# Intelligent-Microsystems-Lab/SNNQuantPrune

Hardware: AMD Instinct MI355X
Metric: samples/sec/node (DVS128 T=20, 4-bit/90%-pruned) (higher is better)
Workload: dtype fp6*fp4->f32 (integer-exact); 1 GPU; C3 topology: 3x(qconv3x3+BN+LIF+pool2) + qdense(32768->110)+LIF + vote, DVS128 128x128x2, T=20, bits 4/4/4/4, 90% pruned; batch_per_gpu=1024, global_batch=1024, frames=20, parallelism=dp1 (batch-sharded, all-gather logits)

## Files before the change

### include/snnqp.h

```cpp
#ifndef SNNQP_H_
#define SNNQP_H_

#include <stdint.h>

#ifdef __cplusplus
extern "C" {
#endif

typedef void *snnqp_stream_t;

enum {
  SNNQP_OK = 0,
  SNNQP_EINVAL = -1,
  SNNQP_EUNSUPPORTED = -2,
  SNNQP_EHIP = -3
};

enum { SNNQP_F32 = 0, SNNQP_U8 = 1, SNNQP_BITS = 2, SNNQP_EV1 = 3, SNNQP_EV4 = 4 };
enum { SNNQP_W_F32 = 0, SNNQP_W_I8 = 1 };
enum {
  SNNQP_NEURON_NONE = 0,
  SNNQP_NEURON_MULTI_STEP_LIF = 1,
  SNNQP_NEURON_PARAMETRIC_LEAKY_IF = 2,
  SNNQP_NEURON_LIF = 3
// ... 73 lines not shown
  int32_t pad_lo[3], pad_hi[3];
  int32_t in_dil[3];
  int32_t k_dil[3];
  int32_t groups;
} snnqp_conv3d_geom_t;

#define SNNQP_VERSION 507
int snnqp_version(void);
const char *snnqp_last_error(void);
const char *snnqp_build_flags(void);

int snnqp_set_conv_k16(int enabled);
int snnqp_set_event_half_group(int enabled);
int snnqp_conv_event_half_group(int in_type, int32_t T, const snnqp_conv_geom_t *g, const snnqp_weight_t *w,
                                const snnqp_neuron_t *nrn, int has_state, int pool, int x_max);

int snnqp_conv_out_shape(const snnqp_conv_geom_t *g, int32_t *OH, int32_t *OW);

int snnqp_quantize(int kind, const float *w, const float *mask, int64_t n,
                   int bits, float p0, float p1, float *fq_out,
                   int8_t *codes_out, int32_t *flags, snnqp_stream_t stream);
int snnqp_quantize_ex(int kind, const float *w, const float *mask, int64_t n,
                      int bits, int sign, float p0, float p1, float *fq_out,
                      int8_t *codes_out, int32_t *flags, snnqp_stream_t stream);

int snnqp_pack_codes_mfma(const int8_t *w, int64_t K, int32_t N, int32_t Npad,
                          int8_t *wt, snnqp_stream_t stream);

int snnqp_pack_codes_fp6(const int8_t *w, int64_t K, int32_t N, int32_t Npad, void *wt6,
                         snnqp_stream_t stream);
// ... 234 lines not shown
```

### snnquantprune_amd/_lib.py

```python

from __future__ import annotations

import ctypes
import os
from ctypes import (POINTER, Structure, c_char_p, c_float, c_int, c_int8,
                    c_int32, c_uint32, c_int64, c_void_p)

_HERE = os.path.dirname(os.path.abspath(__file__))
LIB_PATH = os.path.join(_HERE, "csrc", "libsnnqp.so")

ABI_VERSION = 507

F32, U8, BITS, EV1, EV4 = 0, 1, 2, 3, 4
W_F32, W_I8 = 0, 1
NEURON_NONE, NEURON_MULTI_STEP_LIF, NEURON_PARAMETRIC_LEAKY_IF, NEURON_LIF = 0, 1, 2, 3
SURR_FAST_SIGMOID, SURR_ATAN, SURR_SLAYER, SURR_SMOOTH_STEP, SURR_PIECEWISE_LINEAR = 0, 1, 2, 3, 4
Q_DUQ, Q_UNIFORM_STATIC, Q_PARAMETRIC_D, Q_PARAMETRIC_D_XMAX = 0, 1, 2, 3
IMPL_AUTO, IMPL_GENERIC, IMPL_MFMA = 0, 1, 2
FLAG_CODE_OVERFLOW, FLAG_MASK_NOT_BINARY = 1, 2
FLAG_NOT_INTEGER, FLAG_GT_ONE, FLAG_GT_127, FLAG_GT_15 = 4, 8, 16, 32
OK, EINVAL, EUNSUPPORTED, EHIP = 0, -1, -2, -3
STATUS_QUEUE_CORRUPT, STATUS_TICKET, STATUS_BOUND = 1, 2, 4


# ... 25 lines not shown

class Conv3dGeomT(Structure):
  _fields_ = ([(n, c_int32) for n in ("D", "H", "W", "Cin", "Cout", "KD", "KH", "KW")]
              + [(n, c_int32 * 3) for n in ("stride", "pad_lo", "pad_hi", "in_dil", "k_dil")]
              + [("groups", c_int32)])


_PROTOTYPES = {
    "snnqp_version": (c_int, []),
    "snnqp_last_error": (c_char_p, []),
    "snnqp_build_flags": (c_char_p, []),
    "snnqp_set_conv_k16": (c_int, [c_int]),
    "snnqp_set_event_half_group": (c_int, [c_int]),
    "snnqp_conv_event_half_group": (c_int, [c_int, c_int32, POINTER(ConvGeomT), POINTER(WeightT),
                                            POINTER(NeuronT), c_int, c_int, c_int]),
    "snnqp_conv_out_shape": (c_int, [POINTER(ConvGeomT), POINTER(c_int32),
                                     POINTER(c_int32)]),
    "snnqp_quantize": (c_int, [c_int, c_void_p, c_void_p, c_int64, c_int, c_float,
                               c_float, c_void_p, c_void_p, c_void_p, c_void_p]),
    "snnqp_quantize_ex": (c_int, [c_int, c_void_p, c_void_p, c_int64, c_int, c_int, c_float,
                                  c_float, c_void_p, c_void_p, c_void_p, c_void_p]),
    "snnqp_pack_codes_mfma": (c_int, [c_void_p, c_int64, c_int32, c_int32, c_void_p,
                                      c_void_p]),
    "snnqp_pack_codes_fp6": (c_int, [c_void_p, c_int64, c_int32, c_int32, c_void_p, c_void_p]),
    "snnqp_inspect_f32": (c_int, [c_void_p, c_int64, c_void_p, c_void_p]),
    "snnqp_inspect_u8": (c_int, [c_void_p, c_int64, c_void_p, c_void_p]),
    "snnqp_f32_to_u8": (c_int, [c_void_p, c_void_p, c_int64, c_void_p]),
    "snnqp_narrow_f32": (c_int, [c_void_p, c_void_p, c_int64, c_void_p, c_void_p]),
    "snnqp_pack_frames": (c_int, [c_void_p, c_int64, c_int32, c_int32, c_int, c_void_p, c_void_p,
                                  c_void_p]),
# ... 179 lines not shown
```

### snnquantprune_amd/csrc/api.hip

```cpp
#include <atomic>

#include "common.h"

namespace snnqp {

static std::atomic<int> g_conv_k16{1};
bool conv_k16_enabled() { return g_conv_k16.load(std::memory_order_relaxed) != 0; }
static std::atomic<int> g_event_half_group{1};
bool event_half_group_enabled() { return g_event_half_group.load(std::memory_order_relaxed) != 0; }

static thread_local std::string g_last_error;

void set_error(const char *fmt, ...) {
  char buf[512];
  va_list ap;
  va_start(ap, fmt);
  vsnprintf(buf, sizeof(buf), fmt, ap);
  va_end(ap);
  g_last_error = buf;
}

}

extern "C" {
// ... 5 lines not shown
#ifndef SNNQP_BUILD_FLAGS
#define SNNQP_BUILD_FLAGS ""
#endif
const char *snnqp_build_flags(void) { return SNNQP_BUILD_FLAGS; }

int snnqp_set_conv_k16(int enabled) {
  if (enabled < 0) return snnqp::conv_k16_enabled() ? 1 : 0;
  return snnqp::g_conv_k16.exchange(enabled ? 1 : 0, std::memory_order_relaxed);
}

int snnqp_set_event_half_group(int enabled) {
  if (enabled < 0) return snnqp::event_half_group_enabled() ? 1 : 0;
  return snnqp::g_event_half_group.exchange(enabled ? 1 : 0, std::memory_order_relaxed);
}

int snnqp_conv_out_shape(const snnqp_conv_geom_t *g, int32_t *OH, int32_t *OW) {
  SNNQP_REQUIRE(g && OH && OW, SNNQP_EINVAL, "conv_out_shape: null argument");
  SNNQP_REQUIRE(g->stride_h > 0 && g->stride_w > 0 && g->in_dil_h > 0 &&
                    g->in_dil_w > 0 && g->k_dil_h > 0 && g->k_dil_w > 0 &&
                    g->KH > 0 && g->KW > 0,
                SNNQP_EINVAL, "conv_out_shape: non-positive stride/dilation/kernel");
  const int64_t hd = g->H > 0 ? (int64_t)(g->H - 1) * g->in_dil_h + 1 : 0;
  const int64_t wd = g->W > 0 ? (int64_t)(g->W - 1) * g->in_dil_w + 1 : 0;
  const int64_t kh = (int64_t)(g->KH - 1) * g->k_dil_h + 1;
  const int64_t kw = (int64_t)(g->KW - 1) * g->k_dil_w + 1;
  const int64_t th = hd + g->pad_h_lo + g->pad_h_hi;
  const int64_t tw = wd + g->pad_w_lo + g->pad_w_hi;
  *OH = th < kh ? 0 : (int32_t)((th - kh) / g->stride_h + 1);
  *OW = tw < kw ? 0 : (int32_t)((tw - kw) / g->stride_w + 1);
  return SNNQP_OK;
// ... 4 lines not shown
```

### snnquantprune_amd/csrc/blocks.hip

```cpp
#include "common.h"
#include "kernels.h"

#include <atomic>
#include <cstdlib>
#include <cstring>
#include <mutex>

using namespace snnqp;

namespace {
std::atomic<int64_t> g_fallback_conv{0}, g_fallback_dense{0};
std::mutex g_fallback_mu;
char g_fallback_reason[256] = "";

void note_fallback(bool dense, const char *why) {
  (dense ? g_fallback_dense : g_fallback_conv).fetch_add(1, std::memory_order_relaxed);
  static const bool log = std::getenv("SNNQP_LOG_FALLBACKS") != nullptr;
  std::lock_guard<std::mutex> lock(g_fallback_mu);
  const bool fresh = std::strncmp(g_fallback_reason + (dense ? 7 : 6), why ? why : "", 200) != 0;
  std::snprintf(g_fallback_reason, sizeof(g_fallback_reason), "%s%s", dense ? "dense: " : "conv: ",
                why ? why : "");
  if (log && fresh)
    std::fprintf(stderr, "libsnnqp: %s block on the direct-form kernel: %s\n",
                 dense ? "dense" : "conv", why ? why : "");
// ... 65 lines not shown
  }
  return SNNQP_OK;
}

int snnqp_conv_dequant_form(const snnqp_weight_t *w, const snnqp_neuron_t *nrn) {
  SNNQP_REQUIRE(w && nrn, SNNQP_EINVAL, "conv_dequant_form: null descriptor");
  SNNQP_REQUIRE(w->wtype == SNNQP_W_I8, SNNQP_EINVAL, "conv_dequant_form: int8 codes only");
  return conv3x3_bits_dequant_form(w, nrn);
}

int snnqp_conv_event_half_group(int in_type, int32_t T, const snnqp_conv_geom_t *g, const snnqp_weight_t *w,
                                const snnqp_neuron_t *nrn, int has_state, int pool, int x_max) {
  SNNQP_REQUIRE(g && w && nrn, SNNQP_EINVAL, "conv_event_half_group: null descriptor");
  SNNQP_CHECK_NEURON_KIND(nrn, "conv_event_half_group");
  return conv3x3_event_half_group(in_type, T, g, w, nrn, has_state != 0, pool, x_max);
}

int snnqp_conv_lif_forward(const void *x, int in_type, int64_t x_stride_t,
                           int64_t x_stride_b, int32_t T, int32_t B,
                           const snnqp_conv_geom_t *g, const snnqp_weight_t *w,
                           const int8_t *wt, const snnqp_bn_t *bn,
                           const snnqp_neuron_t *nrn,
                           const float *u0, float *u_out, void *s_out,
                           int s_type, int pool, int impl, int x_max, int32_t *x_seen,
                           int32_t *x_flags, snnqp_stream_t stream) {
  const BlockCall c{x, in_type, x_stride_t, x_stride_b, T, B, w, wt, bn, nrn, u0, u_out, s_out, s_type,
                    x_flags, nullptr, (hipStream_t)stream, g, pool, x_max, x_seen};
  if (int rc = conv_preamble("conv_lif_forward", c, false, true)) return rc;
  SNNQP_REQUIRE(impl >= SNNQP_IMPL_AUTO && impl <= SNNQP_IMPL_MFMA, SNNQP_EINVAL,
                "conv_lif_forward: unknown impl %d", impl);
// ... 122 lines not shown
```

### snnquantprune_amd/csrc/conv3x3_u8c2.hip

```cpp
#include <type_traits>

#include "conv_tile.h"

namespace snnqp {

constexpr int HROW2 = 24;
constexpr int HCOPY2 = HALO * HROW2;
constexpr int HCONST2 = 2 * HCOPY2;
constexpr int HIMG2 = 496;
constexpr int TCHUNK = 32;
constexpr int U8C2_WPS = 4;
constexpr int STG_N = TCHUNK / 2;

typedef int v2i_a4 __attribute__((ext_vector_type(2), aligned(4)));
typedef __attribute__((address_space(3))) const v2i_a4 lds_cv2i_t;

__host__ __device__ inline int u8c2_table_bytes(int lutm, int bound, int rows) {
  const int b = lutm == LUT_CHANNEL ? rows * 128 : lutm == LUT_SHARED ? (2 * bound + 2) * 4 : 0;
  return (b + 15) & ~15;
}

#ifndef SNNQP_U8C2_EV1_WPS
#define SNNQP_U8C2_EV1_WPS 5
#endif
#ifndef SNNQP_U8C2_ONE_WPS
#define SNNQP_U8C2_ONE_WPS 4
#endif
#ifndef SNNQP_U8C2_EV1_ONE_WPS
#define SNNQP_U8C2_EV1_ONE_WPS 6
#endif
template <int NF, bool POOL, int LUTM, int IN, bool ONE>
constexpr int u8c2_waves() {
  if (IN == SNNQP_EV1 && ONE && LUTM == LUT_CHANNEL && NF == NF_MUL0 && POOL) return SNNQP_U8C2_EV1_ONE_WPS;
  if (IN == SNNQP_EV1) return SNNQP_U8C2_EV1_WPS;
  return ONE ? SNNQP_U8C2_ONE_WPS : U8C2_WPS;
}
template <int NF, bool POOL, int LUTM, int IN = SNNQP_U8, bool ONE = false, bool HALF = false>
__global__ void __launch_bounds__(256, (u8c2_waves<NF, POOL, LUTM, IN, ONE>()))
conv3x3_u8c2_kernel(ConvMfmaArgs a) {
  constexpr int FL = OutStage<POOL>::FL;
  constexpr bool EV1 = IN == SNNQP_EV1;
  static_assert(!HALF || (EV1 && ONE && LUTM == LUT_CHANNEL && NF == NF_MUL0),
                "the half group: bit-packed frames, one chunk, per-channel tables, NF_MUL0");
  constexpr bool EV4 = IN == SNNQP_EV4;
  constexpr bool F32IN = IN == SNNQP_F32;
  static_assert(TCHUNK % FL == 0, "flush period must divide the staging chunk");
  if constexpr (!EV1) {
    if (a.pred && *(const volatile int32_t *)a.pred == 0) return;
  }
  extern __shared__ __attribute__((aligned(16))) uint8_t lds[];
  const int tc = a.tchunk;
  const int lut_off = tc * HIMG2;
  uint32_t *obuf = (uint32_t *)(lds + lut_off + u8c2_table_bytes(LUTM, a.lut_bound, a.lut_rows));
  const int tid = threadIdx.x, lane = tid & 63;
  const int wave = __builtin_amdgcn_readfirstlane(tid >> 6);
  const int n = lane & 31, h = lane >> 5;
  const int cout_base = blockIdx.y * 128 + wave * 32;
  const bool wave_on = cout_base < a.Cout;
  const int cout = wave_on ? cout_base + n : n;
  const int cpar = cout < a.Cout ? cout : a.Cout - 1;
  const uint32_t cmask = chan_mask(cout_base, a.cout_fire);
  const bool half_wave = HALF && cout_base + 32 == a.Cout;
  const int ctab = half_wave && n >= 16 ? cout - 16 : cout;
  uint32_t *wgw = obuf + OutStage<POOL>::BYTES / 4;
  if (tid == 0) { wgw[0] = 0x7F800000u; wgw[1] = 0u; }
  typedef int v2i_a8 __attribute__((ext_vector_type(2)));
  v2i_a8 *xtab = (v2i_a8 *)(wgw + 4);
  if (EV1) {
    const uint32_t one = LUTM == LUT_CHANNEL ? 16u : LUTM == LUT_SHARED ? 4u : 0x81u;
    const uint32_t zero = LUTM == LUT_NONE ? 0x80u : 0u;
    uint32_t e[2] = {0, 0};
#pragma unroll
    for (int j = 0; j < 8; ++j) e[j >> 2] |= (((uint32_t)tid >> j) & 1u ? one : zero) << (8 * (j & 3));
    xtab[tid] = v2i_a8{(int)e[0], (int)e[1]};
  }
  if (LUTM != LUT_NONE) lds_barrier();
  if (LUTM == LUT_SHARED) {
    build_lut((float *)(lds + lut_off), a.lut_bound, a.dq, tid);
    if (NF == NF_MUL0) {
      lds_barrier();
      atomicMin(wgw, lut_bn_min_bits((const float *)(lds + lut_off), a.lut_bound, a.bn,
                                     blockIdx.y * 128, a.Cout, tid, 256));
    }
  }
  int ch_row0 = 0, ch_col = 0;
  if (LUTM == LUT_CHANNEL) {
    int pos = 0, neg = 0;
#pragma unroll
    for (int j = 0; j < 16; ++j) {
      const int k = 16 * h + j, dy = k >> 3, b = k & 7;
      if (k < 24 && b < 6 && wave_on && cout < a.Cout) {
        const int code = a.w[(int64_t)(6 * dy + b) * a.Cout + ctab];
        pos += code > 0 ? code : 0;
        neg += code < 0 ? -code : 0;
      }
    }
    pos += __shfl_xor(pos, 32);
    neg += __shfl_xor(neg, 32);
    uint32_t *scr = obuf;
    int slot = 4 * n + wave;
    if (a.ch_slots) slot = a.ch_slots[blockIdx.y * 128 + wave * 32 + n] & 127;
    if (h == 0) {
      scr[slot] = (uint32_t)((pos + neg) * a.x_limit + 1);
      scr[128 + wave * 32 + n] = (uint32_t)(neg * a.x_limit);
      scr[256 + wave * 32 + n] = (uint32_t)slot;
    }
    lds_barrier();
    ch_col = slot >> 2;
    const int start = lut_column_start(scr, slot);
    int total = 0;
#pragma unroll
    for (int k = 0; k < 4; ++k) total += (int)scr[(slot & ~3) + k];
    ch_row0 = start + neg * a.x_limit;
    if (total > a.lut_rows && a.status) *(volatile uint32_t *)a.status = SNNQP_STATUS_BOUND;
    const uint32_t mb = build_lut_channel<HALF>((float *)(lds + lut_off), scr, a.lut_rows, a.dq, a.bn,
                                                blockIdx.y * 128, a.Cout, tid);
    atomicMin(wgw, mb);
    lds_barrier();
  }
  if (tid < tc) {
    *(uint32_t *)(lds + tid * HIMG2 + HCONST2) = 0x7F7F7F7Fu;
    *(uint32_t *)(lds + tid * HIMG2 + HCONST2 + 4) = 0x00000001u;
  }

  float acc_off = 0.0f;
  int tab0 = 0;
  v4i bf, bfg;
  {
    int bias = 0;
    if (LUTM == LUT_SHARED) bias = (int)lds_addr(lds) + lut_off + 4 * a.lut_bound;
    if (LUTM == LUT_CHANNEL)
      bias = (int)lds_addr(lds) + lut_off + 4 * (ch_row0 * 32 + ch_col);
    if (HALF) tab0 = bias;
    int q = bias / 127;
    const int r = bias - 127 * q;
    int wsum = 0;
    int v[4], vg[4];
#pragma unroll
    for (int d = 0; d < 4; ++d) {
      uint32_t pk = 0, pkg = 0;
#pragma unroll
      for (int j = 0; j < 4; ++j) {
        const int k = 16 * h + 4 * d + j;
// ... 24 lines not shown
      vg[d] = (int)pkg;
    }
    bf = v4i{v[0], v[1], v[2], v[3]};
    bfg = v4i{vg[0], vg[1], vg[2], vg[3]};
    acc_off = 128.0f * (float)(wsum + __shfl_xor(wsum, 32));
  }

  LaneConsts lc = {0.f, 1.f, 0.f, 0.f, a.nrn.vr};
  if (a.bn.mean) { lc.bmean = a.bn.mean[cpar]; lc.bmul = a.bn.mul[cpar]; lc.bbias = a.bn.bias[cpar]; }
  if (a.nrn.kind == SNNQP_NEURON_LIF) lc.dec = a.nrn.decay[cpar];

  const int ty = ((n >> 2) & 1) | ((n >> 4) << 1);
  const int tx = (n & 3) | (((n >> 3) & 1) << 2);
  const int cpy = tx & 1;
  const int px0 = (int)lds_addr(lds) + cpy * HCOPY2 + 2 * tx + 2 * cpy;
  const int tyh = half_wave ? 2 * ty : ty;
  int offA[2], offB[2];
#pragma unroll
  for (int tl = 0; tl < 2; ++tl) {
    offA[tl] = px0 + (tyh + 4 * tl + (h ? 2 : 0)) * HROW2;
    offB[tl] = h ? (int)lds_addr(lds) + HCONST2 : px0 + (ty + 4 * tl + 1) * HROW2;
  }
  if (HALF && half_wave) offB[1] = tab0;
  const uint8_t *xb = (const uint8_t *)a.x;
  const int ob0 = (half_wave ? lane : out_pix<POOL>(0, lane)) * 4 + wave;
  const int ob1 = out_pix<POOL>(1, lane) * 4 + wave;
  const bool store_lane = POOL ? lane < (half_wave ? 16 : 8) : (half_wave || lane < 32);
  uint32_t seen = 0;
  uint32_t hist[6] = {0, 0, 0, 0, 0, 0};
  const int s_pix = tid & 127;
  const bool s_task = s_pix < HALO * HALO;
  const int s_half = __builtin_amdgcn_readfirstlane(tid >> 7);
  const int s_dst = (s_pix / HALO) * HROW2 + (s_pix % HALO) * 2;

  PatchWalk pw(a);
  int r = __builtin_amdgcn_readfirstlane((int)pw.first);
  uint32_t processed = 0;
  while (r < (int)pw.count) {
    ++processed;
    int claimed = 0;
    if (pw.queue && tid == 0) claimed = (int)pw.claim();
    int b, y0, x0;
// ... 140 lines not shown
            }
            const uint16_t val = (uint16_t)(w2 ^ 0x8080u);
            uint8_t *p = lds + tt * HIMG2 + s_dst;
            *(uint16_t *)p = val;
            *(uint16_t *)(p + HCOPY2 + 2) = val;
          }
        }
        lds_barrier();
      }
      }
      auto run_chunk = [&](auto mode_tag, auto fma_tag) {
      constexpr int MODE = decltype(mode_tag)::value;
      constexpr bool FMA = decltype(fma_tag)::value;
      constexpr bool OFFS = MODE == LUT_NONE;
      const v4i bw = OFFS ? bfg : bf;
      if constexpr (HALF) {
        if (half_wave) {
          int ctab0 = offB[1];
          asm volatile("" : "+v"(ctab0));
          const v16i c0 = splat16(ctab0);
          for (int tf = 0; tf < nt; tf += FL) {
            const int nf = min(FL, nt - tf);
#pragma unroll 1
            for (int tt = tf; tt < tf + nf; ++tt) {
              const uint32_t img = (uint32_t)(tt * HIMG2);
              const v2i_a4 lo = *(lds_cv2i_t *)(uintptr_t)(img + (uint32_t)offA[0]);
              const v2i_a4 hi = *(lds_cv2i_t *)(uintptr_t)(img + (uint32_t)offA[0] + (uint32_t)HROW2);
              const v16i acc = __builtin_amdgcn_mfma_i32_32x32x32_i8(v4i{lo.x, lo.y, hi.x, hi.y}, bw, c0,
                                                                     0, 0, 0);
              const uint32_t word = tile_epilogue_halves<NF, POOL, MODE, FMA, OFFS, true>(
                  acc, u[0], a.dq, lc, a.nrn, lane, acc_off);
              if (store_lane) {
// ... 60 lines not shown
    r = r_next;
  }
  if (a.x_seen && tid == 0) {
    if (seen != 0) atomicMax(a.x_seen, seen);
#pragma unroll
    for (int k = 0; k < 6; ++k)
      if (hist[k] != 0) atomicAdd((uint32_t *)a.x_seen + 1 + k, hist[k]);
  }
  if (pw.queue && tid == 0) pw.finish(processed, a.npatch, a.status);
}


namespace {
struct U8c2Plan {
  int32_t x_limit, lut_bound, lut_rows, tchunk;
  bool lut, lutc, one, half;
  size_t ldsb;
};
U8c2Plan u8c2_plan(int in_type, int32_t T, int32_t Cout, const snnqp_weight_t *w, int nf, bool has_state,
                   bool pl, int x_max) {
  U8c2Plan p;
  const bool ev1 = in_type == SNNQP_EV1;
  const int64_t xm = ev1 ? 1 : (x_max > 0 ? x_max : 1);
  p.x_limit = (int32_t)(xm > 255 ? 255 : xm);
  const int64_t bound = (int64_t)w->abs_sum_max * xm;
  p.lut = w->abs_sum_max > 0 && xm > 0 && xm <= LUT_XMAX && bound <= LUT_CAP;
  p.lut_bound = p.lut ? (int32_t)bound : 0;
  p.tchunk = T >= TCHUNK ? TCHUNK : T;
  const size_t lds_fixed = (size_t)p.tchunk * HIMG2 + 16 + (ev1 ? 2048 : 0) +
                           (pl ? OutStage<true>::BYTES : OutStage<false>::BYTES);
  const int64_t stack = w->ch_stack_max > 0 ? (int64_t)w->ch_stack_max : 8 * (int64_t)w->abs_sum_max;
// ... 3 lines not shown
  const int lm = p.lutc ? LUT_CHANNEL : p.lut ? LUT_SHARED : LUT_NONE;
  const size_t lds_rest = lds_fixed - (size_t)p.tchunk * HIMG2 + u8c2_table_bytes(lm, p.lut_bound, p.lut_rows);
  for (int wgs = 4; wgs >= 2; --wgs) {
    const size_t per_wg = (size_t)(160 * 1024) / wgs - 512;
    int tc = p.tchunk;
    while (tc > 16 && (size_t)tc * HIMG2 + lds_rest > per_wg) tc -= 1;
    if ((size_t)tc * HIMG2 + lds_rest <= per_wg) {
      p.tchunk = tc;
      break;
    }
  }
  p.ldsb = (size_t)p.tchunk * HIMG2 + lds_rest;
  p.one = !has_state && T <= p.tchunk;
  p.half = event_half_group_enabled() && ev1 && p.one && p.lutc && nf == NF_MUL0 && w->cout_fire > 0 &&
           w->cout_fire % 16 == 0 && w->cout_fire + 16 == Cout && Cout % 32 == 0;
  return p;
}
}

int conv3x3_event_half_group(int in_type, int32_t T, const snnqp_conv_geom_t *g, const snnqp_weight_t *w,
                             const snnqp_neuron_t *nrn, bool has_state, int pool, int x_max) {
  SNNQP_REQUIRE(g && w && nrn, SNNQP_EINVAL, "conv_event_half_group: null descriptor");
  SNNQP_REQUIRE(pool == 1 || pool == 2, SNNQP_EINVAL, "conv_event_half_group: pool must be 1 or 2");
  SNNQP_REQUIRE(T >= 0, SNNQP_EINVAL, "conv_event_half_group: negative T");
  if (in_type != SNNQP_EV1 || T == 0) return 0;
  BlockCall c;
  c.in_type = in_type; c.g = g; c.w = w; c.nrn = nrn;
  if (conv3x3_mfma_unsupported(c)) return 0;
  SNNQP_REQUIRE(w->L >= 1.0f, SNNQP_EINVAL, "dequant L must be >= 1");
  if (int rc = conv3x3_check_cout_fire("conv_event_half_group", w, g->Cout)) return rc;
  return u8c2_plan(in_type, T, g->Cout, w, neuron_form(make_neuron(nrn)), has_state, pool == 2, x_max).half ? 1 : 0;
}

template <int NF, int LUTM, int IN>
static void launch_u8c2_pool(const ConvMfmaArgs &a, bool pool, bool one, unsigned gy, hipStream_t st, size_t lds) {
  if (pool && one) launch_persistent(conv3x3_u8c2_kernel<NF, true, LUTM, IN, true>, a, gy, st, lds);
  else if (pool) launch_persistent(conv3x3_u8c2_kernel<NF, true, LUTM, IN>, a, gy, st, lds);
  else if (one) launch_persistent(conv3x3_u8c2_kernel<NF, false, LUTM, IN, true>, a, gy, st, lds);
  else launch_persistent(conv3x3_u8c2_kernel<NF, false, LUTM, IN>, a, gy, st, lds);
}

template <int NF, int LUTM>
static void launch_u8c2_in(const ConvMfmaArgs &a, int in_type, bool pool, bool one, unsigned gy, hipStream_t st,
                           size_t lds) {
  if (in_type == SNNQP_EV1) launch_u8c2_pool<NF, LUTM, SNNQP_EV1>(a, pool, one, gy, st, lds);
  else if (in_type == SNNQP_EV4) launch_u8c2_pool<NF, LUTM, SNNQP_EV4>(a, pool, one, gy, st, lds);
// ... 20 lines not shown
  const unsigned gy = (unsigned)((a.Cout + 127) / 128);
  const U8c2Plan plan = u8c2_plan(in_type, a.T, a.Cout, w, nf, a.u0 || a.u_out, pl, x_max);
  a.x_limit = plan.x_limit;
  a.lut_bound = plan.lut_bound;
  a.tchunk = plan.tchunk;
  a.lut_rows = plan.lut_rows;
  a.ch_slots = plan.lutc && w->ch_stack_max > 0 ? w->ch_slots : nullptr;
  a.cout_fire = w->cout_fire > 0 ? w->cout_fire : a.Cout;
  if (in_type == SNNQP_F32) {
    SNNQP_REQUIRE(x_flags != nullptr && (((uintptr_t)a.x) & 7) == 0 && a.xs_t % 2 == 0 && a.xs_b % 2 == 0,
                  SNNQP_EINVAL, "conv3x3 mfma: float32 frames need x_flags and 8-byte aligned pixels");
    if (int rc = zero_words_async((uint32_t *)x_flags, 1, st)) return rc;
    a.x_flags = x_flags;
  }
  if (plan.lut) check_code_bound_once(stream_device(st), a.w, (int64_t)9 * a.Cin, a.Cout, w->abs_sum_max, st);
  if (plan.half && pl)
    launch_persistent(conv3x3_u8c2_kernel<NF_MUL0, true, LUT_CHANNEL, SNNQP_EV1, true, true>, a, gy, st, plan.ldsb);
  else if (plan.half)
    launch_persistent(conv3x3_u8c2_kernel<NF_MUL0, false, LUT_CHANNEL, SNNQP_EV1, true, true>, a, gy, st, plan.ldsb);
  else if (plan.lutc) launch_u8c2_nf<LUT_CHANNEL>(a, nf, in_type, pl, plan.one, gy, st, plan.ldsb);
  else if (plan.lut) launch_u8c2_nf<LUT_SHARED>(a, nf, in_type, pl, plan.one, gy, st, plan.ldsb);
  else launch_u8c2_nf<LUT_NONE>(a, nf, in_type, pl, plan.one, gy, st, plan.ldsb);
  return SNNQP_OK;
}

}
```

### snnquantprune_amd/csrc/conv_tile.h

```cpp
#pragma once
#include "kernels.h"

namespace snnqp {

struct v2f {
  float x, y;
};
__device__ __forceinline__ v2f operator+(v2f a, v2f b) { return v2f{a.x + b.x, a.y + b.y}; }
__device__ __forceinline__ v2f operator-(v2f a, v2f b) { return v2f{a.x - b.x, a.y - b.y}; }
__device__ __forceinline__ v2f operator*(v2f a, v2f b) { return v2f{a.x * b.x, a.y * b.y}; }
__device__ __forceinline__ v2f operator+(v2f a, float b) { return v2f{a.x + b, a.y + b}; }
__device__ __forceinline__ v2f operator-(v2f a, float b) { return v2f{a.x - b, a.y - b}; }
__device__ __forceinline__ v2f operator*(v2f a, float b) { return v2f{a.x * b, a.y * b}; }
__device__ __forceinline__ v2f operator-(v2f a) { return v2f{-a.x, -a.y}; }
__device__ __forceinline__ v2f fma2(v2f a, v2f b, v2f c) {
  return v2f{__builtin_fmaf(a.x, b.x, c.x), __builtin_fmaf(a.y, b.y, c.y)};
}


enum { LUT_NONE = 0, LUT_SHARED = 1, LUT_CHANNEL = 2 };
constexpr int LUT_CAP = 4095;
constexpr int LUT2_ROWS = 256;
constexpr int LUT_XMAX = 31;

// ... 302 lines not shown
        const uint32_t pw = (uint32_t)o | (uint32_t)(o >> 32);
        myw = writelane_u32(pw, i >> 1, myw);
      } else {
        const int r0 = (i & 3) + 8 * (i >> 2);
        myw = writelane_u32((uint32_t)m0, r0, myw);
        myw = writelane_u32((uint32_t)(m0 >> 32), r0 + 4, myw);
        myw = writelane_u32((uint32_t)m1, r0 + 1, myw);
        myw = writelane_u32((uint32_t)(m1 >> 32), r0 + 5, myw);
      }
    }
    __builtin_amdgcn_sched_barrier(0);
  }
  return myw;
}

template <bool POOL>
struct OutStage {
  static constexpr int NPIX = POOL ? 16 : 64;
  static constexpr int FL = POOL ? 32 : 8;
  static constexpr int BYTES = FL * NPIX * 16;
};

template <bool POOL>
__device__ __forceinline__ int out_pix(int tl, int lane) {
  if (POOL) return (tl * 2 + ((lane >> 2) & 1)) * 4 + (lane & 3);
  const int ty = ((lane >> 2) & 1) | (((lane >> 4) & 1) << 1);
  const int tx = (lane & 3) | (((lane >> 3) & 1) << 2);
  return (tl * 4 + ty) * 8 + tx;
}

// ... 85 lines not shown
  const unsigned gx = persistent_grid((const void *)kernel, threads, dyn_lds, dev, a.npatch, a.B, &a.xcd_split);
  hipLaunchKernelGGL(kernel, dim3(gx, gy), dim3(threads), dyn_lds, st, a);
  if (a.sched) sched_release(dev, slot, st);
}

int conv3x3_check_cout_fire(const char *who, const snnqp_weight_t *w, int32_t Cout);
inline int wt_cin_pad(const snnqp_weight_t *w, int32_t Cin) { return w->wt_cin ? w->wt_cin : (Cin + 31) / 32 * 32; }

enum { DQ_ARITH = 1, DQ_ONE = 2, DQ_TABLE = 3 };
constexpr int DQT_MAXA = 2047;
void launch_conv3x3_bits(ConvMfmaArgs a, const snnqp_weight_t *w, const snnqp_neuron_t *nrn, hipStream_t st);
int launch_conv3x3_u8c2(ConvMfmaArgs a, int in_type, const snnqp_weight_t *w, int x_max, int32_t *x_flags,
                        hipStream_t st);
bool conv_k16_enabled();
bool event_half_group_enabled();

}
```

### snnquantprune_amd/csrc/kernels.h

```cpp
#pragma once
#include "common.h"
#include "tile_util.h"

namespace snnqp {

struct BlockCall {
  const void *x = nullptr;
  int in_type = SNNQP_BITS;
  int64_t xs_t = 0, xs_b = 0;
  int32_t T = 0, B = 0;
  const snnqp_weight_t *w = nullptr;
  const int8_t *wt = nullptr;
  const snnqp_bn_t *bn = nullptr;
  const snnqp_neuron_t *nrn = nullptr;
  const float *u0 = nullptr;
  float *u_out = nullptr;
  void *s_out = nullptr;
  int s_type = SNNQP_BITS;
  int32_t *x_flags = nullptr;
  const int32_t *pred = nullptr;
  hipStream_t st = nullptr;
  const snnqp_conv_geom_t *g = nullptr;
  int pool = 1, x_max = 0;
  int32_t *x_seen = nullptr;
// ... 17 lines not shown
};
int run_generic(const BlockCall &c, int32_t *acc_out, const GenericDepth *dz);

const char *conv3x3_geometry_unsupported(const snnqp_conv_geom_t *g);
const char *conv3x3_mfma_unsupported(const BlockCall &c);
const char *conv3x3_currents_unsupported(int in_type, int64_t NB, const snnqp_conv_geom_t *g,
                                         const snnqp_weight_t *w, const int8_t *wt);
int run_conv3x3_currents(const void *x, int64_t NB, const snnqp_conv_geom_t *g,
                         const snnqp_weight_t *w, const int8_t *wt, float *y, int32_t *acc,
                         hipStream_t st);
int run_current_min(const snnqp_weight_t *w, const snnqp_bn_t *bn, int32_t bound, int32_t Cout,
                    uint32_t *out_bits, hipStream_t st);
int conv3x3_bits_dequant_form(const snnqp_weight_t *w, const snnqp_neuron_t *nrn);
int conv3x3_event_half_group(int in_type, int32_t T, const snnqp_conv_geom_t *g, const snnqp_weight_t *w,
                             const snnqp_neuron_t *nrn, bool has_state, int pool, int x_max);
int run_conv3x3_mfma(const BlockCall &c);

constexpr int MAX_DEVICES = 64;
struct DeviceGuard {
  int prev = -1;
  bool ok = true;
  explicit DeviceGuard(int dev) {
    int cur = -1;
    if (hipGetDevice(&cur) != hipSuccess) { (void)hipGetLastError(); ok = false; return; }
    if (cur == dev) return;
    if (hipSetDevice(dev) != hipSuccess) { (void)hipGetLastError(); ok = false; return; }
    prev = cur;
  }
  ~DeviceGuard() {
    if (prev >= 0 && hipSetDevice(prev) != hipSuccess) (void)hipGetLastError();
// ... 42 lines not shown
```

### snnquantprune_amd/linen.py

```python

from __future__ import annotations

import dataclasses
import functools
import hashlib
import math
import threading
from collections.abc import MutableMapping
from typing import Any, Callable, Dict, Iterable, Optional, Sequence

import torch

_tls = threading.local()


def _stack():
  if not hasattr(_tls, "stack"):
    _tls.stack = []
  return _tls.stack


class ConfigDict(MutableMapping):

  def __init__(self, *args, **kwargs):
# ... 92 lines not shown


def conv_k16() -> bool:
  from . import _lib
  return bool(_lib.lib().snnqp_set_conv_k16(-1))


def set_event_half_group(enabled: bool):
  from . import _lib
  _lib.lib().snnqp_set_event_half_group(1 if enabled else 0)


def event_half_group() -> bool:
  from . import _lib
  return bool(_lib.lib().snnqp_set_event_half_group(-1))


_TRAIN_CONV_MFMA = True


def set_train_conv_mfma(enabled: bool) -> bool:
  global _TRAIN_CONV_MFMA
  old = _TRAIN_CONV_MFMA
  _TRAIN_CONV_MFMA = bool(enabled)
  return old


def train_conv_mfma() -> bool:
  return _TRAIN_CONV_MFMA

# ... 458 lines not shown
```

### snnquantprune_amd/ops.py

```python

from __future__ import annotations

import ctypes
import math
from dataclasses import dataclass
from typing import Optional, Sequence, Tuple

import torch

from . import _lib as L




class PackedSpikes:

  def __init__(self, bits: torch.Tensor, channels: int):
    assert bits.dtype == torch.int32 and bits.is_contiguous()
    assert bits.shape[-1] == (channels + 31) // 32
    self.bits = bits
    self.channels = int(channels)
    self.flat_perm = None
    self.chan_map = None

# ... 935 lines not shown
  dev = xt.device
  u0, u_out, s, spikes = _scan_outputs(dev, (T, B, OH // pool, OW // pool), geom.Cout, u0, want_u, packed_out,
                               state=(B, OH, OW))
  g, w, n = geom.struct(), weight.struct(), neuron.struct()
  b = bn.struct() if bn is not None else None
  cin_l, cout_l = (geom.Cin, geom.Cout) if logical is None else logical[:2]
  tag = "conv%dx%d[%dx%dx%d->%d]" % (geom.KH, geom.KW, geom.H, geom.W, cin_l, cout_l)
  if _PROFILE is not None and in_type == L.BITS and weight.is_int and "dequant" not in PROFILE_NOTES.get(tag, {}):
    PROFILE_NOTES.setdefault(tag, {})["dequant"] = conv_dequant_form(weight, neuron)
  if _PROFILE is not None and logical is not None:
    PROFILE_NOTES.setdefault(tag, {})["channels"] = {
        "cin": geom.Cin, "cout": geom.Cout, "live_out": int(logical[2])}
    if weight.cout_fire and packed_out:
      ev1 = L.EV1 if (in_type == L.EV1 or (binary_first and in_type in (L.U8, L.F32))) else in_type
      PROFILE_NOTES[tag]["channels"]["half_group"] = conv_event_half_group(
          ev1, T, geom, weight, neuron, state=u0 is not None or want_u, pool=pool, x_max=1 if ev1 == L.EV1 else x_max)
  speculate = (binary_first and packed_out and not isinstance(x, (PackedFrames, PackedSpikes))
               and in_type in (L.U8, L.F32) and geom.Cin == 2 and weight.is_int and impl != L.IMPL_GENERIC
               and xt.ndim == 5)
  with _timed(tag):
    if speculate:
      pf, not_binary = pack_frames_checked(xt)
      ps_t, ps_b = _tb_strides(pf.data, T, B, time_major, pf.data.shape[-1])
      try:
        L.check(L.lib().snnqp_conv_lif_forward(
            _ptr(pf.data), L.EV1, ps_t, ps_b, T, B, ctypes.byref(g), ctypes.byref(w),
            _ptr(weight.wt), _ref(b), ctypes.byref(n),
            _ptr(u0), _ptr(u_out), _ptr(s), L.BITS, pool, impl, 1, None, None, _stream()))
      except L.SnnqpError as e:
        if e.code != L.EUNSUPPORTED:
# ... 144 lines not shown
  L.check(L.lib().snnqp_workqueue_stats(ctypes.byref(a), ctypes.byref(b), ctypes.byref(c), 1 if reset else 0))
  return {"captured_static_walks": a.value, "busy_static_walks": b.value, "dequant_table_fallbacks": c.value}


def workqueue_capture_mark(device) -> int:
  m = ctypes.c_int64()
  L.check(L.lib().snnqp_workqueue_capture_mark(int(torch.device(device).index or 0), ctypes.byref(m)))
  return int(m.value)


def workqueue_capture_release(device, begin: int, end: int):
  L.check(L.lib().snnqp_workqueue_capture_release(int(torch.device(device).index or 0), int(begin), int(end)))


DQ_FORMS = {1: "arith", 2: "one", 3: "table"}


def conv_event_half_group(in_type: int, T: int, geom: ConvGeom, w: Weight, nrn: Neuron, state: bool = False,
                          pool: int = 1, x_max: int = 0) -> bool:
  gs, ws, ns = geom.struct(), w.struct(), nrn.struct()
  rc = L.lib().snnqp_conv_event_half_group(int(in_type), int(T), ctypes.byref(gs), ctypes.byref(ws),
                                           ctypes.byref(ns), 1 if state else 0, int(pool), int(x_max))
  if rc < 0:
    L.check(rc)
  return rc == 1


def conv_dequant_form(w: Weight, nrn: Neuron) -> str:
  ws, ns = w.struct(), nrn.struct()
  rc = L.lib().snnqp_conv_dequant_form(ctypes.byref(ws), ctypes.byref(ns))
# ... 494 lines not shown
```

Measured before the change: 98080 samples/s.

## Spread first-layer event conv work across all waves instead of idling tail waves

Adds a 'wave spread' variant of the bit-packed-frame first conv kernel. When Cout is 64, or 96 with the half group, each wave pair now covers one 32-channel group and splits the two row tiles between its two waves. The extra 16-channel half group is also split into quarter tiles across all four waves, so no wave idles or loops twice. The intent is to balance MFMA and epilogue work across waves in the CTA, removing the imbalance where the half wave did double work. The cost is extra per-wave weight-fragment construction, a new quarter epilogue, and a different occupancy bound.

```diff
diff --git a/include/snnqp.h b/include/snnqp.h
--- a/include/snnqp.h
+++ b/include/snnqp.h
@@ -111,6 +111,9 @@
 int snnqp_set_event_half_group(int enabled);
 int snnqp_conv_event_half_group(int in_type, int32_t T, const snnqp_conv_geom_t *g, const snnqp_weight_t *w,
                                 const snnqp_neuron_t *nrn, int has_state, int pool, int x_max);
+int snnqp_set_event_wave_spread(int enabled);
+int snnqp_conv_event_wave_spread(int in_type, int32_t T, const snnqp_conv_geom_t *g, const snnqp_weight_t *w,
+                                 const snnqp_neuron_t *nrn, int has_state, int pool, int x_max);
 
 int snnqp_conv_out_shape(const snnqp_conv_geom_t *g, int32_t *OH, int32_t *OW);
 
diff --git a/snnquantprune_amd/_lib.py b/snnquantprune_amd/_lib.py
--- a/snnquantprune_amd/_lib.py
+++ b/snnquantprune_amd/_lib.py
@@ -63,6 +63,9 @@
     "snnqp_set_event_half_group": (c_int, [c_int]),
     "snnqp_conv_event_half_group": (c_int, [c_int, c_int32, POINTER(ConvGeomT), POINTER(WeightT),
                                             POINTER(NeuronT), c_int, c_int, c_int]),
+    "snnqp_set_event_wave_spread": (c_int, [c_int]),
+    "snnqp_conv_event_wave_spread": (c_int, [c_int, c_int32, POINTER(ConvGeomT), POINTER(WeightT),
+                                             POINTER(NeuronT), c_int, c_int, c_int]),
     "snnqp_conv_out_shape": (c_int, [POINTER(ConvGeomT), POINTER(c_int32),
                                      POINTER(c_int32)]),
     "snnqp_quantize": (c_int, [c_int, c_void_p, c_void_p, c_int64, c_int, c_float,
diff --git a/snnquantprune_amd/csrc/api.hip b/snnquantprune_amd/csrc/api.hip
--- a/snnquantprune_amd/csrc/api.hip
+++ b/snnquantprune_amd/csrc/api.hip
@@ -8,6 +8,8 @@
 bool conv_k16_enabled() { return g_conv_k16.load(std::memory_order_relaxed) != 0; }
 static std::atomic<int> g_event_half_group{1};
 bool event_half_group_enabled() { return g_event_half_group.load(std::memory_order_relaxed) != 0; }
+static std::atomic<int> g_event_wave_spread{1};
+bool event_wave_spread_enabled() { return g_event_wave_spread.load(std::memory_order_relaxed) != 0; }
 
 static thread_local std::string g_last_error;
 
@@ -43,6 +45,11 @@
   return snnqp::g_event_half_group.exchange(enabled ? 1 : 0, std::memory_order_relaxed);
 }
 
+int snnqp_set_event_wave_spread(int enabled) {
+  if (enabled < 0) return snnqp::event_wave_spread_enabled() ? 1 : 0;
+  return snnqp::g_event_wave_spread.exchange(enabled ? 1 : 0, std::memory_order_relaxed);
+}
+
 int snnqp_conv_out_shape(const snnqp_conv_geom_t *g, int32_t *OH, int32_t *OW) {
   SNNQP_REQUIRE(g && OH && OW, SNNQP_EINVAL, "conv_out_shape: null argument");
   SNNQP_REQUIRE(g->stride_h > 0 && g->stride_w > 0 && g->in_dil_h > 0 &&
diff --git a/snnquantprune_amd/csrc/blocks.hip b/snnquantprune_amd/csrc/blocks.hip
--- a/snnquantprune_amd/csrc/blocks.hip
+++ b/snnquantprune_amd/csrc/blocks.hip
@@ -103,6 +103,13 @@
   SNNQP_REQUIRE(g && w && nrn, SNNQP_EINVAL, "conv_event_half_group: null descriptor");
   SNNQP_CHECK_NEURON_KIND(nrn, "conv_event_half_group");
   return conv3x3_event_half_group(in_type, T, g, w, nrn, has_state != 0, pool, x_max);
+}
+
+int snnqp_conv_event_wave_spread(int in_type, int32_t T, const snnqp_conv_geom_t *g, const snnqp_weight_t *w,
+                                 const snnqp_neuron_t *nrn, int has_state, int pool, int x_max) {
+  SNNQP_REQUIRE(g && w && nrn, SNNQP_EINVAL, "conv_event_wave_spread: null descriptor");
+  SNNQP_CHECK_NEURON_KIND(nrn, "conv_event_wave_spread");
+  return conv3x3_event_wave_spread(in_type, T, g, w, nrn, has_state != 0, pool, x_max);
 }
 
 int snnqp_conv_lif_forward(const void *x, int in_type, int64_t x_stride_t,
diff --git a/snnquantprune_amd/csrc/conv3x3_u8c2.hip b/snnquantprune_amd/csrc/conv3x3_u8c2.hip
--- a/snnquantprune_amd/csrc/conv3x3_u8c2.hip
+++ b/snnquantprune_amd/csrc/conv3x3_u8c2.hip
@@ -29,19 +29,23 @@
 #ifndef SNNQP_U8C2_EV1_ONE_WPS
 #define SNNQP_U8C2_EV1_ONE_WPS 6
 #endif
-template <int NF, bool POOL, int LUTM, int IN, bool ONE>
+#ifndef SNNQP_U8C2_SPREAD_WPS
+#define SNNQP_U8C2_SPREAD_WPS 6
+#endif
+template <int NF, bool POOL, int LUTM, int IN, bool ONE, bool SPREAD = false>
 constexpr int u8c2_waves() {
+  if (SPREAD && POOL) return SNNQP_U8C2_SPREAD_WPS;
   if (IN == SNNQP_EV1 && ONE && LUTM == LUT_CHANNEL && NF == NF_MUL0 && POOL) return SNNQP_U8C2_EV1_ONE_WPS;
   if (IN == SNNQP_EV1) return SNNQP_U8C2_EV1_WPS;
   return ONE ? SNNQP_U8C2_ONE_WPS : U8C2_WPS;
 }
-template <int NF, bool POOL, int LUTM, int IN = SNNQP_U8, bool ONE = false, bool HALF = false>
-__global__ void __launch_bounds__(256, (u8c2_waves<NF, POOL, LUTM, IN, ONE>()))
+template <int NF, bool POOL, int LUTM, int IN = SNNQP_U8, bool ONE = false, bool HALF = false, bool SPREAD = false>
+__global__ void __launch_bounds__(256, (u8c2_waves<NF, POOL, LUTM, IN, ONE, SPREAD>()))
 conv3x3_u8c2_kernel(ConvMfmaArgs a) {
   constexpr int FL = OutStage<POOL>::FL;
   constexpr bool EV1 = IN == SNNQP_EV1;
-  static_assert(!HALF || (EV1 && ONE && LUTM == LUT_CHANNEL && NF == NF_MUL0),
-                "the half group: bit-packed frames, one chunk, per-channel tables, NF_MUL0");
+  static_assert(!(HALF || SPREAD) || (EV1 && ONE && LUTM == LUT_CHANNEL && NF == NF_MUL0),
+                "the half group, the wave spread: bit-packed frames, one chunk, per-channel tables, NF_MUL0");
   constexpr bool EV4 = IN == SNNQP_EV4;
   constexpr bool F32IN = IN == SNNQP_F32;
   static_assert(TCHUNK % FL == 0, "flush period must divide the staging chunk");
@@ -59,7 +63,7 @@
   const bool wave_on = cout_base < a.Cout;
   const int cout = wave_on ? cout_base + n : n;
   const int cpar = cout < a.Cout ? cout : a.Cout - 1;
-  const uint32_t cmask = chan_mask(cout_base, a.cout_fire);
+  uint32_t cmask = chan_mask(cout_base, a.cout_fire);
   const bool half_wave = HALF && cout_base + 32 == a.Cout;
   const int ctab = half_wave && n >= 16 ? cout - 16 : cout;
   uint32_t *wgw = obuf + OutStage<POOL>::BYTES / 4;
@@ -84,6 +88,7 @@
     }
   }
   int ch_row0 = 0, ch_col = 0;
+  int hg_row0 = 0, hg_col = 0;
   if (LUTM == LUT_CHANNEL) {
     int pos = 0, neg = 0;
 #pragma unroll
@@ -112,6 +117,16 @@
 #pragma unroll
     for (int k = 0; k < 4; ++k) total += (int)scr[(slot & ~3) + k];
     ch_row0 = start + neg * a.x_limit;
+    if constexpr (SPREAD) {
+      auto entry_of = [&](int grp, int &row0, int &col) {
+        int s = 4 * n + grp;
+        if (a.ch_slots) s = a.ch_slots[blockIdx.y * 128 + grp * 32 + n] & 127;
+        row0 = lut_column_start(scr, s) + (int)scr[128 + grp * 32 + n];
+        col = s >> 2;
+      };
+      entry_of(wave >> 1, ch_row0, ch_col);
+      if (HALF) entry_of(2, hg_row0, hg_col);
+    }
     if (total > a.lut_rows && a.status) *(volatile uint32_t *)a.status = SNNQP_STATUS_BOUND;
     const uint32_t mb = build_lut_channel<HALF>((float *)(lds + lut_off), scr, a.lut_rows, a.dq, a.bn,
                                                 blockIdx.y * 128, a.Cout, tid);
@@ -126,7 +141,43 @@
   float acc_off = 0.0f;
   int tab0 = 0;
   v4i bf, bfg;
-  {
+  v4i bfh = {0, 0, 0, 0};
+  if constexpr (SPREAD) {
+    auto taps = [&](int chan, int shift, bool all_taps, int bias) {
+      int q = bias / 127;
+      const int r = bias - 127 * q;
+      int v[4];
+#pragma unroll
+      for (int d = 0; d < 4; ++d) {
+        uint32_t pk = 0;
+#pragma unroll
+        for (int j = 0; j < 4; ++j) {
+          const int k = 16 * h + 4 * d + j, kk = k - shift;
+          uint32_t bv = 0;
+          if (all_taps || k < 24) {
+            if (kk >= 0 && kk < 24 && (kk & 7) < 6)
+              bv = (uint8_t)(a.w[(int64_t)(6 * (kk >> 3) + (kk & 7)) * a.Cout + chan] * 8);
+          } else if (k < 28) {
+            const int part = q < 127 ? q : 127;
+            q -= part;
+            bv = (uint32_t)part;
+          } else if (k == 28) {
+            bv = (uint32_t)r;
+          }
+          pk |= bv << (8 * j);
+        }
+        v[d] = (int)pk;
+      }
+      return v4i{v[0], v[1], v[2], v[3]};
+    };
+    const int tbase = (int)lds_addr(lds) + lut_off;
+    bf = taps(blockIdx.y * 128 + (wave >> 1) * 32 + n, 0, false, tbase + 4 * (ch_row0 * 32 + ch_col));
+    bfg = bf;
+    if (HALF) {
+      tab0 = tbase + 4 * (hg_row0 * 32 + hg_col);
+      bfh = taps(blockIdx.y * 128 + 64 + (n & 15), n >= 16 ? 8 : 0, true, 0);
+    }
+  } else {
     int bias = 0;
     if (LUTM == LUT_SHARED) bias = (int)lds_addr(lds) + lut_off + 4 * a.lut_bound;
     if (LUTM == LUT_CHANNEL)
@@ -181,18 +232,39 @@
   const int tx = (n & 3) | (((n >> 3) & 1) << 2);
   const int cpy = tx & 1;
   const int px0 = (int)lds_addr(lds) + cpy * HCOPY2 + 2 * tx + 2 * cpy;
-  const int tyh = half_wave ? 2 * ty : ty;
+  const bool half_loop = half_wave && !SPREAD;
+  const int tyh = half_loop ? 2 * ty : ty;
   int offA[2], offB[2];
 #pragma unroll
   for (int tl = 0; tl < 2; ++tl) {
     offA[tl] = px0 + (tyh + 4 * tl + (h ? 2 : 0)) * HROW2;
     offB[tl] = h ? (int)lds_addr(lds) + HCONST2 : px0 + (ty + 4 * tl + 1) * HROW2;
   }
-  if (HALF && half_wave) offB[1] = tab0;
+  if (HALF && half_loop) offB[1] = tab0;
   const uint8_t *xb = (const uint8_t *)a.x;
-  const int ob0 = (half_wave ? lane : out_pix<POOL>(0, lane)) * 4 + wave;
-  const int ob1 = out_pix<POOL>(1, lane) * 4 + wave;
-  const bool store_lane = POOL ? lane < (half_wave ? 16 : 8) : (half_wave || lane < 32);
+  int ob0 = (half_loop ? lane : out_pix<POOL>(0, lane)) * 4 + wave;
+  int ob1 = out_pix<POOL>(1, lane) * 4 + wave;
+  const bool store_lane = POOL ? lane < (half_loop ? 16 : 8) : (half_loop || lane < 32);
+  bool quarter_lane = false;
+  uint32_t qmask = 0u;
+  if constexpr (SPREAD) {
+    const int g = wave >> 1, q = wave & 1;
+    offA[0] = q ? offA[1] : offA[0];
+    offB[0] = q ? offB[1] : offB[0];
+    ob0 = out_pix<POOL>(q, lane) * 4 + g;
+    cmask = chan_mask(blockIdx.y * 128 + g * 32, a.cout_fire);
+    if (HALF) {
+      const int np = n ^ (8 * wave);
+      const int typ = ((np >> 2) & 1) | ((np >> 4) << 1), txp = (np & 3) | (((np >> 3) & 1) << 2);
+      offA[1] = (int)lds_addr(lds) + cpy * HCOPY2 + 2 * txp + 2 * cpy + (2 * typ + 2 * h) * HROW2;
+      offB[1] = tab0;
+      const int pix = POOL ? (2 * g + ((lane >> 2) & 1)) * 4 + 2 * q + (lane & 1)
+                           : (4 * g + ((lane >> 2) & 3)) * 8 + 4 * q + (lane & 3);
+      ob1 = pix * 4 + 2;
+      quarter_lane = POOL ? lane < 8 && (lane & 2) == 0 : lane < 16;
+      qmask = chan_mask(blockIdx.y * 128 + 64, a.cout_fire);
+    }
+  }
   uint32_t seen = 0;
   uint32_t hist[6] = {0, 0, 0, 0, 0, 0};
   const int s_pix = tid & 127;
@@ -363,8 +435,44 @@
       constexpr bool FMA = decltype(fma_tag)::value;
       constexpr bool OFFS = MODE == LUT_NONE;
       const v4i bw = OFFS ? bfg : bf;
+      if constexpr (SPREAD) {
+        int ctab0 = offB[1];
+        asm volatile("" : "+v"(ctab0));
+        const v4i c4 = {ctab0, ctab0, ctab0, ctab0};
+        const v16i c0 = __builtin_shufflevector(c4, c4, 0, 1, 2, 3, -1, -1, -1, -1, -1, -1, -1, -1, -1, -1, -1, -1);
+        for (int tf = 0; tf < nt; tf += FL) {
+          const int nf = min(FL, nt - tf);
+#pragma unroll 1
+          for (int tt = tf; tt < tf + nf; ++tt) {
+            const uint32_t img = (uint32_t)(tt * HIMG2);
+            uint32_t *o = obuf + ((t0 + tt) % FL) * (OutStage<POOL>::NPIX * 4);
+            {
+              const v2i_a4 lo = *(lds_cv2i_t *)(uintptr_t)(img + (uint32_t)offA[0]);
+              const v2i_a4 hi = *(lds_cv2i_t *)(uintptr_t)(img + (uint32_t)offB[0]);
+              v16i acc = splat16(0);
+              acc = __builtin_amdgcn_mfma_i32_32x32x32_i8(v4i{lo.x, lo.y, hi.x, hi.y}, bw, acc, 0, 0, 0);
+              const uint32_t word = tile_epilogue_halves<NF, POOL, MODE, FMA, OFFS>(acc, u[0], a.dq, lc, a.nrn,
+                                                                                    lane, acc_off);
+              if (store_lane) o[ob0] = word & cmask;
+            }
+            if constexpr (HALF) {
+              const v2i_a4 lo = *(lds_cv2i_t *)(uintptr_t)(img + (uint32_t)offA[1]);
+              const v2i_a4 hi = *(lds_cv2i_t *)(uintptr_t)(img + (uint32_t)offA[1] + (uint32_t)HROW2);
+              const v16i acc = __builtin_amdgcn_mfma_i32_32x32x32_i8(v4i{lo.x, lo.y, hi.x, hi.y}, bfh, c0,
+                                                                     0, 0, 0);
+              const uint32_t word = tile_epilogue_quarter<NF, POOL, MODE, FMA, OFFS>(acc, u[1], a.dq, lc, a.nrn,
+                                                                                     acc_off);
+              if (quarter_lane) o[ob1] = word & qmask;
+            }
+          }
+          lds_barrier();
+          flush_out<POOL>(obuf, a, t0 + tf, nf, b, y0, x0, tid);
+          lds_barrier();
+        }
+        return;
+      }
       if constexpr (HALF) {
-        if (half_wave) {
+        if (half_loop) {
           int ctab0 = offB[1];
           asm volatile("" : "+v"(ctab0));
           const v16i c0 = splat16(ctab0);
@@ -455,7 +563,7 @@
 namespace {
 struct U8c2Plan {
   int32_t x_limit, lut_bound, lut_rows, tchunk;
-  bool lut, lutc, one, half;
+  bool lut, lutc, one, half, spread;
   size_t ldsb;
 };
 U8c2Plan u8c2_plan(int in_type, int32_t T, int32_t Cout, const snnqp_weight_t *w, int nf, bool has_state,
@@ -489,22 +597,34 @@
   p.one = !has_state && T <= p.tchunk;
   p.half = event_half_group_enabled() && ev1 && p.one && p.lutc && nf == NF_MUL0 && w->cout_fire > 0 &&
            w->cout_fire % 16 == 0 && w->cout_fire + 16 == Cout && Cout % 32 == 0;
+  p.spread = event_wave_spread_enabled() && ev1 && p.one && p.lutc && nf == NF_MUL0 &&
+             (p.half ? Cout == 96 : Cout == 64);
   return p;
 }
 }
 
-int conv3x3_event_half_group(int in_type, int32_t T, const snnqp_conv_geom_t *g, const snnqp_weight_t *w,
-                             const snnqp_neuron_t *nrn, bool has_state, int pool, int x_max) {
-  SNNQP_REQUIRE(g && w && nrn, SNNQP_EINVAL, "conv_event_half_group: null descriptor");
-  SNNQP_REQUIRE(pool == 1 || pool == 2, SNNQP_EINVAL, "conv_event_half_group: pool must be 1 or 2");
-  SNNQP_REQUIRE(T >= 0, SNNQP_EINVAL, "conv_event_half_group: negative T");
+static int event_plan_flag(const char *who, bool U8c2Plan::*flag, int in_type, int32_t T, const snnqp_conv_geom_t *g,
+                           const snnqp_weight_t *w, const snnqp_neuron_t *nrn, bool has_state, int pool, int x_max) {
+  SNNQP_REQUIRE(g && w && nrn, SNNQP_EINVAL, "%s: null descriptor", who);
+  SNNQP_REQUIRE(pool == 1 || pool == 2, SNNQP_EINVAL, "%s: pool must be 1 or 2", who);
+  SNNQP_REQUIRE(T >= 0, SNNQP_EINVAL, "%s: negative T", who);
   if (in_type != SNNQP_EV1 || T == 0) return 0;
   BlockCall c;
   c.in_type = in_type; c.g = g; c.w = w; c.nrn = nrn;
   if (conv3x3_mfma_unsupported(c)) return 0;
   SNNQP_REQUIRE(w->L >= 1.0f, SNNQP_EINVAL, "dequant L must be >= 1");
-  if (int rc = conv3x3_check_cout_fire("conv_event_half_group", w, g->Cout)) return rc;
-  return u8c2_plan(in_type, T, g->Cout, w, neuron_form(make_neuron(nrn)), has_state, pool == 2, x_max).half ? 1 : 0;
+  if (int rc = conv3x3_check_cout_fire(who, w, g->Cout)) return rc;
+  return u8c2_plan(in_type, T, g->Cout, w, neuron_form(make_neuron(nrn)), has_state, pool == 2, x_max).*flag ? 1 : 0;
+}
+
+int conv3x3_event_half_group(int in_type, int32_t T, const snnqp_conv_geom_t *g, const snnqp_weight_t *w,
+                             const snnqp_neuron_t *nrn, bool has_state, int pool, int x_max) {
+  return event_plan_flag("conv_event_half_group", &U8c2Plan::half, in_type, T, g, w, nrn, has_state, pool, x_max);
+}
+
+int conv3x3_event_wave_spread(int in_type, int32_t T, const snnqp_conv_geom_t *g, const snnqp_weight_t *w,
+                              const snnqp_neuron_t *nrn, bool has_state, int pool, int x_max) {
+  return event_plan_flag("conv_event_wave_spread", &U8c2Plan::spread, in_type, T, g, w, nrn, has_state, pool, x_max);
 }
 
 template <int NF, int LUTM, int IN>
@@ -555,7 +675,13 @@
     a.x_flags = x_flags;
   }
   if (plan.lut) check_code_bound_once(stream_device(st), a.w, (int64_t)9 * a.Cin, a.Cout, w->abs_sum_max, st);
-  if (plan.half && pl)
+  if (plan.spread) {
+    constexpr int N0 = NF_MUL0, LC = LUT_CHANNEL, E1 = SNNQP_EV1;
+    if (plan.half && pl) launch_persistent(conv3x3_u8c2_kernel<N0, true, LC, E1, true, true, true>, a, gy, st, plan.ldsb);
+    else if (plan.half) launch_persistent(conv3x3_u8c2_kernel<N0, false, LC, E1, true, true, true>, a, gy, st, plan.ldsb);
+    else if (pl) launch_persistent(conv3x3_u8c2_kernel<N0, true, LC, E1, true, false, true>, a, gy, st, plan.ldsb);
+    else launch_persistent(conv3x3_u8c2_kernel<N0, false, LC, E1, true, false, true>, a, gy, st, plan.ldsb);
+  } else if (plan.half && pl)
     launch_persistent(conv3x3_u8c2_kernel<NF_MUL0, true, LUT_CHANNEL, SNNQP_EV1, true, true>, a, gy, st, plan.ldsb);
   else if (plan.half)
     launch_persistent(conv3x3_u8c2_kernel<NF_MUL0, false, LUT_CHANNEL, SNNQP_EV1, true, true>, a, gy, st, plan.ldsb);
diff --git a/snnquantprune_amd/csrc/conv_tile.h b/snnquantprune_amd/csrc/conv_tile.h
--- a/snnquantprune_amd/csrc/conv_tile.h
+++ b/snnquantprune_amd/csrc/conv_tile.h
@@ -340,6 +340,34 @@
   return myw;
 }
 
+template <int NF, bool POOL, int LUTM, bool FMA = false, bool OFFS = false>
+__device__ __forceinline__ uint32_t tile_epilogue_quarter(const v16i &acc, float (&u)[16], const Dequant &dq,
+                                                          const LaneConsts &lc, const NeuronP &nrn,
+                                                          float off = 0.0f) {
+  uint32_t myw = 0;
+  v2f y[2];
+#pragma unroll
+  for (int j = 0; j < 2; ++j) y[j] = dequant_pair<LUTM, OFFS>(acc[2 * j], acc[2 * j + 1], dq, off);
+#pragma unroll
+  for (int j = 0; j < 2; ++j) {
+    unsigned long long m0, m1;
+    neuron_pair<NF, LUTM == LUT_CHANNEL, FMA>(y[j], u[2 * j], u[2 * j + 1], lc, nrn, m0, m1);
+    if (POOL) {
+      const unsigned long long o = m0 | m1;
+      const uint32_t lo = (uint32_t)o, hi = (uint32_t)(o >> 32);
+      myw = writelane_u32((lo | (lo >> 16)) & 0xFFFFu, j, myw);
+      myw = writelane_u32((hi | (hi >> 16)) & 0xFFFFu, 4 + j, myw);
+    } else {
+#pragma unroll
+      for (int r = 0; r < 4; ++r) {
+        myw = writelane_u32((uint32_t)(m0 >> (16 * r)) & 0xFFFFu, 4 * r + 2 * j, myw);
+        myw = writelane_u32((uint32_t)(m1 >> (16 * r)) & 0xFFFFu, 4 * r + 2 * j + 1, myw);
+      }
+    }
+  }
+  return myw;
+}
+
 template <bool POOL>
 struct OutStage {
   static constexpr int NPIX = POOL ? 16 : 64;
@@ -455,5 +483,6 @@
                         hipStream_t st);
 bool conv_k16_enabled();
 bool event_half_group_enabled();
-
-}
+bool event_wave_spread_enabled();
+
+}
diff --git a/snnquantprune_amd/csrc/kernels.h b/snnquantprune_amd/csrc/kernels.h
--- a/snnquantprune_amd/csrc/kernels.h
+++ b/snnquantprune_amd/csrc/kernels.h
@@ -55,6 +55,8 @@
 int conv3x3_bits_dequant_form(const snnqp_weight_t *w, const snnqp_neuron_t *nrn);
 int conv3x3_event_half_group(int in_type, int32_t T, const snnqp_conv_geom_t *g, const snnqp_weight_t *w,
                              const snnqp_neuron_t *nrn, bool has_state, int pool, int x_max);
+int conv3x3_event_wave_spread(int in_type, int32_t T, const snnqp_conv_geom_t *g, const snnqp_weight_t *w,
+                              const snnqp_neuron_t *nrn, bool has_state, int pool, int x_max);
 int run_conv3x3_mfma(const BlockCall &c);
 
 constexpr int MAX_DEVICES = 64;
diff --git a/snnquantprune_amd/linen.py b/snnquantprune_amd/linen.py
--- a/snnquantprune_amd/linen.py
+++ b/snnquantprune_amd/linen.py
@@ -130,6 +130,16 @@
 def event_half_group() -> bool:
   from . import _lib
   return bool(_lib.lib().snnqp_set_event_half_group(-1))
+
+
+def set_event_wave_spread(enabled: bool):
+  from . import _lib
+  _lib.lib().snnqp_set_event_wave_spread(1 if enabled else 0)
+
+
+def event_wave_spread() -> bool:
+  from . import _lib
+  return bool(_lib.lib().snnqp_set_event_wave_spread(-1))
 
 
 _TRAIN_CONV_MFMA = True
diff --git a/snnquantprune_amd/ops.py b/snnquantprune_amd/ops.py
--- a/snnquantprune_amd/ops.py
+++ b/snnquantprune_amd/ops.py
@@ -973,6 +973,8 @@
     if weight.cout_fire and packed_out:
       ev1 = L.EV1 if (in_type == L.EV1 or (binary_first and in_type in (L.U8, L.F32))) else in_type
       PROFILE_NOTES[tag]["channels"]["half_group"] = conv_event_half_group(
+          ev1, T, geom, weight, neuron, state=u0 is not None or want_u, pool=pool, x_max=1 if ev1 == L.EV1 else x_max)
+      PROFILE_NOTES[tag]["channels"]["wave_spread"] = conv_event_wave_spread(
           ev1, T, geom, weight, neuron, state=u0 is not None or want_u, pool=pool, x_max=1 if ev1 == L.EV1 else x_max)
   speculate = (binary_first and packed_out and not isinstance(x, (PackedFrames, PackedSpikes))
                and in_type in (L.U8, L.F32) and geom.Cin == 2 and weight.is_int and impl != L.IMPL_GENERIC
@@ -1147,6 +1149,16 @@
 
 
 DQ_FORMS = {1: "arith", 2: "one", 3: "table"}
+
+
+def conv_event_wave_spread(in_type: int, T: int, geom: ConvGeom, w: Weight, nrn: Neuron, state: bool = False,
+                           pool: int = 1, x_max: int = 0) -> bool:
+  gs, ws, ns = geom.struct(), w.struct(), nrn.struct()
+  rc = L.lib().snnqp_conv_event_wave_spread(int(in_type), int(T), ctypes.byref(gs), ctypes.byref(ws),
+                                            ctypes.byref(ns), 1 if state else 0, int(pool), int(x_max))
+  if rc < 0:
+    L.check(rc)
+  return rc == 1
 
 
 def conv_event_half_group(in_type: int, T: int, geom: ConvGeom, w: Weight, nrn: Neuron, state: bool = False,
```

Measured after the change: 103,600 samples/s, median of 6. +5.6%, better.
